# JeffreyXiang/ivid

Measured on NVIDIA H100. Metric: 128x128 RGBD multiview samples/sec, higher is better.
Workload: dtype fp16 tensor-core operands, fp32 accumulate / residual stream / GroupNorm / softmax / sampler

## Files before the change

ivid_b200/csrc/common.cuh:

```cuda
#pragma once
#include <cuda.h>
#include <cuda_fp16.h>
#include <cuda_fp8.h>
#include <cuda_runtime.h>
#include <stdint.h>

namespace ivid {

__device__ __forceinline__ uint32_t smem_u32(const void* p) {
  return static_cast<uint32_t>(__cvta_generic_to_shared(p));
}

__device__ __forceinline__ float silu_f(float x) {
  float e, r;
  asm("ex2.approx.ftz.f32 %0, %1;" : "=f"(e) : "f"(x * -1.4426950408889634f));
  asm("rcp.approx.ftz.f32 %0, %1;" : "=f"(r) : "f"(1.0f + e));
  return x * r;
}

__device__ __forceinline__ __half split_term(float v, int seg) {
  const __half hi = __float2half_rn(v);
  return seg == 1 ? __float2half_rn(v - __half2float(hi)) : hi;
}

// ... 34 lines not shown
    if (++spins > IVID_MBAR_SPIN_LIMIT) { __trap(); }
  }
}

__device__ __forceinline__ void bulk_load_1d(void* dst, const void* src, uint32_t bytes, uint64_t* bar) {
  asm volatile("cp.async.bulk.shared::cluster.global.mbarrier::complete_tx::bytes [%0], [%1], %2, [%3];\n" ::"r"(smem_u32(dst)),
               "l"(src), "r"(bytes), "r"(smem_u32(bar))
               : "memory");
}

__device__ __forceinline__ void tma_prefetch_desc(const CUtensorMap* m) {
  asm volatile("prefetch.tensormap [%0];\n" ::"l"(reinterpret_cast<uint64_t>(m)) : "memory");
}
__device__ __forceinline__ void tma_load_2d(const CUtensorMap* m, uint64_t* bar, void* dst, int c0, int c1) {
  asm volatile(
      "cp.async.bulk.tensor.2d.shared::cluster.global.mbarrier::complete_tx::bytes [%0], [%1, {%3, %4}], [%2];\n"
      ::"r"(smem_u32(dst)), "l"(reinterpret_cast<uint64_t>(m)), "r"(smem_u32(bar)), "r"(c0), "r"(c1)
      : "memory");
}
__device__ __forceinline__ void tma_load_3d(const CUtensorMap* m, uint64_t* bar, void* dst, int c0, int c1, int c2) {
  asm volatile(
      "cp.async.bulk.tensor.3d.shared::cluster.global.mbarrier::complete_tx::bytes [%0], [%1, {%3, %4, %5}], [%2];\n"
      ::"r"(smem_u32(dst)), "l"(reinterpret_cast<uint64_t>(m)), "r"(smem_u32(bar)), "r"(c0), "r"(c1), "r"(c2)
      : "memory");
}
__device__ __forceinline__ void tma_load_4d(const CUtensorMap* m, uint64_t* bar, void* dst, int c0, int c1, int c2,
                                            int c3) {
  asm volatile(
      "cp.async.bulk.tensor.4d.shared::cluster.global.mbarrier::complete_tx::bytes [%0], [%1, {%3, %4, %5, %6}], "
      "[%2];\n" ::"r"(smem_u32(dst)),
      "l"(reinterpret_cast<uint64_t>(m)), "r"(smem_u32(bar)), "r"(c0), "r"(c1), "r"(c2), "r"(c3)
      : "memory");
}

__device__ __forceinline__ void wgmma_fence() { asm volatile("wgmma.fence.sync.aligned;\n" ::: "memory"); }
__device__ __forceinline__ void wgmma_commit() { asm volatile("wgmma.commit_group.sync.aligned;\n" ::: "memory"); }
template <int kPending>
__device__ __forceinline__ void wgmma_wait() { asm volatile("wgmma.wait_group.sync.aligned %0;\n" ::"n"(kPending) : "memory"); }
template <int R>
__device__ __forceinline__ void reg_fence(float (&d)[R]) {
#pragma unroll
  for (int i = 0; i < R; ++i) asm volatile("" : "+f"(d[i])::"memory");
}

__device__ __forceinline__ uint64_t make_smem_desc_sw128(uint32_t smem_addr, uint32_t sbo_bytes, uint32_t lbo_bytes) {
  uint64_t d = 0;
  d |= static_cast<uint64_t>((smem_addr & 0x3FFFF) >> 4);
  d |= static_cast<uint64_t>((lbo_bytes >> 4) & 0x3FFF) << 16;
  d |= static_cast<uint64_t>((sbo_bytes >> 4) & 0x3FFF) << 32;
  d |= static_cast<uint64_t>(1) << 62;
  return d;
}

template <int N>
__device__ void wgmma_ss(float (&d)[N / 2], uint64_t desc_a, uint64_t desc_b, uint32_t scale_d);
template <int N>
__device__ void wgmma_rs_tb(float (&d)[N / 2], const uint32_t (&a)[4], uint64_t desc_b, uint32_t scale_d);
template <>
__device__ __forceinline__ void wgmma_ss<16>(float (&d)[8], uint64_t desc_a, uint64_t desc_b, uint32_t scale_d) {
  asm volatile(
      "{\n\t.reg .pred p;\n\tsetp.ne.b32 p, %10, 0;\n\t"
      "wgmma.mma_async.sync.aligned.m64n16k16.f32.f16.f16 {%0, %1, %2, %3, %4, %5, %6, %7}, %8, %9, p, 1, 1, 0, 0;\n\t}\n"
      : "+f"(d[0]), "+f"(d[1]), "+f"(d[2]), "+f"(d[3]), "+f"(d[4]), "+f"(d[5]), "+f"(d[6]), "+f"(d[7])
      : "l"(desc_a), "l"(desc_b), "r"(scale_d));
}
template <>
// ... 64 lines not shown
```

ivid_b200/csrc/conv_gemm.cuh:

```cuda
#pragma once
#include <type_traits>

#include "common.cuh"

namespace ivid {

struct ConvGemmParams {
  int N, H, W;
  int TW, TH, TN;
  int tiles_w, tiles_h, tiles_n;
  int n_blocks;
  int seg_chunks[3];
  int seg_taps[3];
  int Cout;
  int ldc;
  int ldr;
  int out_mode;
  const float* bias;
  const float* residual;
  int res_up;
  void* out;
  __half* out16;
  double* stats;
  float acc_scale;
};

struct ConvMaps {
  CUtensorMap a[3];
  CUtensorMap b;
};
struct ConvMaps8 : ConvMaps {
  CUtensorMap b8;
};

template <int BN, bool SLAB = false>
struct ConvGemmCfg {
  static constexpr int BM = 128;
  static constexpr int BK = 64;
  static constexpr int A_BYTES = BM * BK * 2;
  static constexpr int B_BYTES = ((BN * BK * 2 + 1023) / 1024) * 1024;
  static constexpr int STAGE_BYTES = A_BYTES + B_BYTES;
  static constexpr int STAGES = BN == 128 && !SLAB ? 3 : 4;
  static constexpr int SLAB_BYTES = 16 * 10 * 128;
  static constexpr int SLAB_STAGES = 2;
  static constexpr int RING_BYTES = SLAB ? SLAB_STAGES * SLAB_BYTES + STAGES * B_BYTES : STAGES * STAGE_BYTES;
  static constexpr int BAR_BYTES = 128;
  static constexpr int STAT_BYTES = 8 * 2 * BN * 4;
  static constexpr bool STATS_ON_RING = SLAB;
  static constexpr int SMEM_BYTES = RING_BYTES + BAR_BYTES + (STATS_ON_RING ? 0 : STAT_BYTES) + 1024;
  static constexpr int CONSUMER_THREADS = 256;
  static constexpr int THREADS = CONSUMER_THREADS + 32;
};

struct ConvKCursor {
  int seg = 0, t = 0, ch = 0, base = 0;
};

template <int BN, bool A8 = false, bool SLAB = false>
__global__ void __launch_bounds__(ConvGemmCfg<BN>::THREADS, 2)
conv_gemm_kernel(const __grid_constant__ std::conditional_t<A8, ConvMaps8, ConvMaps> maps, const __grid_constant__ ConvGemmParams p) {
  using Cfg = ConvGemmCfg<BN, SLAB>;
  constexpr int STAGES = Cfg::STAGES;
  constexpr int SLAB_STAGES = Cfg::SLAB_STAGES;
  extern __shared__ uint8_t smem_raw[];
  uint8_t* smem = smem_raw + ((1024u - (smem_u32(smem_raw) & 1023u)) & 1023u);
  uint64_t* full_bar = reinterpret_cast<uint64_t*>(smem + Cfg::RING_BYTES);
  uint64_t* empty_bar = full_bar + STAGES;
  uint64_t* slab_full = empty_bar + STAGES;
  uint64_t* slab_empty = slab_full + SLAB_STAGES;
  float* stat_smem = reinterpret_cast<float*>(Cfg::STATS_ON_RING ? smem : smem + Cfg::RING_BYTES + Cfg::BAR_BYTES);
  uint8_t* const slab_ring = smem;
  uint8_t* const w_ring = smem + SLAB_STAGES * Cfg::SLAB_BYTES;

  const int tid = threadIdx.x;
  const int warp = tid >> 5, lane = tid & 31;
  const int wg = warp >> 2;

  if (tid == 0) {
    for (int s = 0; s < STAGES; ++s) {
      mbar_init(&full_bar[s], 1);
      mbar_init(&empty_bar[s], 8u);
    }
    if constexpr (SLAB) {
      for (int s = 0; s < SLAB_STAGES; ++s) {
        mbar_init(&slab_full[s], 1);
        mbar_init(&slab_empty[s], 8u);
      }
    }
    fence_barrier_init();
  }
  __syncthreads();

  int nunits = 0;
  for (int sg = 0; sg < 3; ++sg) nunits += p.seg_chunks[sg] * p.seg_taps[sg];
  const int nunits8 = A8 ? p.seg_chunks[0] * p.seg_taps[0] : 0;

  const int mt = static_cast<int>(blockIdx.x) / p.n_blocks, nb = static_cast<int>(blockIdx.x) % p.n_blocks;
  const int colbase = nb * BN;
  const int tiles_per_img = p.tiles_w * p.tiles_h;
  const int tn = mt / tiles_per_img;
  const int rem = mt - tn * tiles_per_img;
  const int th = rem / p.tiles_w;
  const int tw = rem - th * p.tiles_w;
  const int n0 = tn * p.TN, h0 = th * p.TH, w0 = tw * p.TW;

  if (warp == Cfg::CONSUMER_THREADS / 32) {
    if (lane == 0) {
      tma_prefetch_desc(&maps.a[0]);
      tma_prefetch_desc(&maps.b);
      if constexpr (A8) tma_prefetch_desc(&maps.b8);
      if constexpr (SLAB) {
        const uint32_t slab_bytes = static_cast<uint32_t>(p.TW * (p.TH + 2)) * 128u;
        uint32_t u = 0, a = 0;
        int base = 0;
#pragma unroll 1
        for (int sg = 0; sg < 3; ++sg) {
          const int chunks = p.seg_chunks[sg];
          const int nx = p.seg_taps[sg] == 9 ? 3 : 1;
          const bool e4m3 = A8 && sg == 0;
#pragma unroll 1
          for (int ch = 0; ch < chunks; ++ch) {
#pragma unroll 1
            for (int xi = 0; xi < nx; ++xi, ++a) {
              const int sl = static_cast<int>(a % SLAB_STAGES);
              if (a >= SLAB_STAGES) mbar_wait(&slab_empty[sl], ((a / SLAB_STAGES) - 1) & 1);
              mbar_arrive_expect_tx(&slab_full[sl], nx == 3 ? slab_bytes : static_cast<uint32_t>(Cfg::A_BYTES));
              tma_load_4d(&maps.a[sg], &slab_full[sl], slab_ring + sl * Cfg::SLAB_BYTES, ch * (e4m3 ? 128 : 64),
                          w0 + (nx == 3 ? xi - 1 : 0), h0 - (nx == 3 ? 1 : 0), n0);
#pragma unroll 1
              for (int yi = 0; yi < nx; ++yi, ++u) {
                const int s = static_cast<int>(u % STAGES);
                if (u >= STAGES) mbar_wait(&empty_bar[s], ((u / STAGES) - 1) & 1);
                mbar_arrive_expect_tx(&full_bar[s], BN * Cfg::BK * 2);
                const int t = nx == 3 ? 3 * yi + xi : 0;
                uint8_t* sb = w_ring + s * Cfg::B_BYTES;
                if constexpr (A8) {
                  if (e4m3) { tma_load_2d(&maps.b8, &full_bar[s], sb, (t * chunks + ch) * 128, colbase); continue; }
                }
                tma_load_2d(&maps.b, &full_bar[s], sb, base + (t * chunks + ch) * 64, colbase);
              }
            }
          }
          if (!e4m3) base += p.seg_taps[sg] * chunks * 64;
// ... 2 lines not shown
        ConvKCursor c;
        while (p.seg_chunks[c.seg] == 0) ++c.seg;
#pragma unroll 1
        for (int u = 0; u < nunits; ++u) {
          const uint32_t g = static_cast<uint32_t>(u);
          const int s = static_cast<int>(g % STAGES);
          if (g >= STAGES) mbar_wait(&empty_bar[s], ((g / STAGES) - 1) & 1);
          const int taps = p.seg_taps[c.seg], chunks = p.seg_chunks[c.seg];
          uint8_t* sa = smem + s * Cfg::STAGE_BYTES;
          uint8_t* sb = sa + Cfg::A_BYTES;
          const int dy = (taps == 9) ? (c.t / 3 - 1) : 0;
          const int dx = (taps == 9) ? (c.t % 3 - 1) : 0;
          mbar_arrive_expect_tx(&full_bar[s], Cfg::A_BYTES + BN * Cfg::BK * 2);
          bool e4m3 = false;
          if constexpr (A8) {
            if (c.seg == 0) {
              tma_load_4d(&maps.a[0], &full_bar[s], sa, c.ch * 128, w0 + dx, h0 + dy, n0);
              tma_load_2d(&maps.b8, &full_bar[s], sb, (c.t * chunks + c.ch) * 128, colbase);
              e4m3 = true;
            }
          }
          if (!e4m3) {
            const int kcol = c.base + (c.t * chunks + c.ch) * 64;
            tma_load_4d(&maps.a[c.seg], &full_bar[s], sa, c.ch * 64, w0 + dx, h0 + dy, n0);
            tma_load_2d(&maps.b, &full_bar[s], sb, kcol, colbase);
          }
          if (++c.ch == chunks) {
            c.ch = 0;
            if (++c.t == taps) { c.t = 0; if (!A8 || c.seg != 0) c.base += taps * chunks * 64; ++c.seg; }
          }
          while (c.seg < 3 && p.seg_chunks[c.seg] == 0) ++c.seg;
        }
      }
    }
    return;
  }

  float acc[BN / 2];
#pragma unroll
  for (int i = 0; i < BN / 2; ++i) acc[i] = 0.f;

  if constexpr (SLAB) {
    const uint32_t row_bytes = static_cast<uint32_t>(p.TW) * 128u;
    uint32_t u = 0, a = 0;
#pragma unroll 1
    for (int sg = 0; sg < 3; ++sg) {
      const int nx = p.seg_taps[sg] == 9 ? 3 : 1;
      const int loads = p.seg_chunks[sg] * nx;
#pragma unroll 1
      for (int l = 0; l < loads; ++l, ++a) {
        const uint32_t sl = a % SLAB_STAGES;
        mbar_wait(&slab_full[sl], (a / SLAB_STAGES) & 1);
        const uint32_t sa = smem_u32(slab_ring + sl * Cfg::SLAB_BYTES) + wg * 64 * 128;
#pragma unroll 1
        for (int yi = 0; yi < nx; ++yi, ++u) {
          const uint32_t s = u % STAGES;
          mbar_wait(&full_bar[s], (u / STAGES) & 1);
          wgmma_fence();
          const uint64_t da = make_smem_desc_sw128(sa + yi * row_bytes, 1024, 16);
          const uint64_t db = make_smem_desc_sw128(smem_u32(w_ring + s * Cfg::B_BYTES), 1024, 16);
          if (A8 && sg == 0) {
#pragma unroll
            for (int k = 0; k < 4; ++k) wgmma_ss_e4m3<BN>(acc, da + 2 * k, db + 2 * k, (u | k) != 0 ? 1u : 0u);
          } else {
#pragma unroll
            for (int k = 0; k < 4; ++k) wgmma_ss<BN>(acc, da + 2 * k, db + 2 * k, (u | k) != 0 ? 1u : 0u);
// ... 12 lines not shown
    if (lane == 0) {
      mbar_arrive(&empty_bar[(u - 1) % STAGES]);
      mbar_arrive(&slab_empty[(a - 1) % SLAB_STAGES]);
    }
  } else {
#pragma unroll 1
    for (int u = 0; u < nunits; ++u) {
      const uint32_t g = static_cast<uint32_t>(u);
      const int s = static_cast<int>(g % STAGES);
      mbar_wait(&full_bar[s], (g / STAGES) & 1);
      const uint32_t sa = smem_u32(smem + s * Cfg::STAGE_BYTES);
      const uint32_t sb = sa + Cfg::A_BYTES;
      wgmma_fence();
      const uint64_t da = make_smem_desc_sw128(sa + wg * 64 * 128, 1024, 16);
      const uint64_t db = make_smem_desc_sw128(sb, 1024, 16);
      if (A8 && u < nunits8) {
#pragma unroll
        for (int k = 0; k < 4; ++k) wgmma_ss_e4m3<BN>(acc, da + 2 * k, db + 2 * k, (u | k) != 0 ? 1u : 0u);
      } else {
#pragma unroll
        for (int k = 0; k < 4; ++k) wgmma_ss<BN>(acc, da + 2 * k, db + 2 * k, (u | k) != 0 ? 1u : 0u);
      }
      wgmma_commit();
      wgmma_wait<1>();
      if (u > 0 && lane == 0) mbar_arrive(&empty_bar[(g - 1) % STAGES]);
    }
    wgmma_wait<0>();
    reg_fence(acc);
    if (lane == 0) mbar_arrive(&empty_bar[static_cast<uint32_t>(nunits - 1) % STAGES]);
  }

  const int wr = warp & 3;
  const int quad = lane & 3;
  uint32_t pix[2], rpix[2];
  bool ok[2];
#pragma unroll
  for (int i = 0; i < 2; ++i) {
    const int row = wg * 64 + wr * 16 + (lane >> 2) + 8 * i;
    const int n = n0 + row / (p.TW * p.TH), h = h0 + (row / p.TW) % p.TH, x = w0 + row % p.TW;
    ok[i] = n < p.N;
    pix[i] = (static_cast<uint32_t>(n) * p.H + h) * p.W + x;
    rpix[i] = p.res_up ? (static_cast<uint32_t>(n) * (p.H >> 1) + (h >> 1)) * (p.W >> 1) + (x >> 1) : pix[i];
  }
  const bool do_stats = p.stats != nullptr;
  if constexpr (Cfg::STATS_ON_RING) {
    if (do_stats) asm volatile("bar.sync 1, %0;\n" ::"n"(Cfg::CONSUMER_THREADS) : "memory");
  }
#pragma unroll
  for (int j = 0; j < BN / 8; ++j) {
    const int c = colbase + 8 * j + 2 * quad;
    float s0 = 0.f, s1 = 0.f, q0 = 0.f, q1 = 0.f;
    if (c < p.Cout) {
      const float2 b = make_float2(__ldg(p.bias + c), __ldg(p.bias + c + 1));
#pragma unroll
      for (int i = 0; i < 2; ++i) {
        if (!ok[i]) continue;
        float v0, v1;
        if (A8) {
          v0 = fmaf(acc[4 * j + 2 * i], p.acc_scale, b.x); v1 = fmaf(acc[4 * j + 2 * i + 1], p.acc_scale, b.y);
        } else {
          v0 = acc[4 * j + 2 * i] + b.x; v1 = acc[4 * j + 2 * i + 1] + b.y;
        }
        if (p.out_mode == 2) {
          const uint32_t hw = static_cast<uint32_t>(p.H) * p.W, n = pix[i] / hw;
          float* o = reinterpret_cast<float*>(p.out) + (static_cast<size_t>(n) * p.Cout + c) * hw + (pix[i] - n * hw);
          o[0] = v0;
          if (c + 1 < p.Cout) o[hw] = v1;
          continue;
        }
        if (p.residual != nullptr) {
          const float2 r = __ldg(reinterpret_cast<const float2*>(p.residual + static_cast<size_t>(rpix[i]) * p.ldr + c));
          v0 += r.x; v1 += r.y;
        }
        if (p.out_mode == 0) {
          *reinterpret_cast<float2*>(reinterpret_cast<float*>(p.out) + static_cast<size_t>(pix[i]) * p.ldc + c) = make_float2(v0, v1);
          if (p.out16 != nullptr) *reinterpret_cast<uint32_t*>(p.out16 + static_cast<size_t>(pix[i]) * p.ldc + c) = pack_h2(v0, v1);
        } else {
          const __half2 hv = __floats2half2_rn(v0, v1);
          *reinterpret_cast<__half2*>(reinterpret_cast<__half*>(p.out) + static_cast<size_t>(pix[i]) * p.ldc + c) = hv;
          const float2 r = __half22float2(hv);
          v0 = r.x; v1 = r.y;
        }
        s0 += v0; s1 += v1;
        q0 = fmaf(v0, v0, q0); q1 = fmaf(v1, v1, q1);
      }
    }
    if (do_stats) {
#pragma unroll
      for (int off = 4; off < 32; off <<= 1) {
        s0 += __shfl_xor_sync(0xffffffffu, s0, off);
        s1 += __shfl_xor_sync(0xffffffffu, s1, off);
        q0 += __shfl_xor_sync(0xffffffffu, q0, off);
        q1 += __shfl_xor_sync(0xffffffffu, q1, off);
      }
      if (lane < 4) {
        float* st = stat_smem + warp * 2 * BN + 8 * j + 2 * quad;
        st[0] = s0; st[1] = s1; st[BN] = q0; st[BN + 1] = q1;
      }
    }
  }
  if (do_stats) {
    asm volatile("bar.sync 1, %0;\n" ::"n"(Cfg::CONSUMER_THREADS) : "memory");
    const int rows_per_n = p.TW * p.TH;
    const int n_tile = (128 + rows_per_n - 1) / rows_per_n;
    for (int e = tid; e < n_tile * BN; e += Cfg::CONSUMER_THREADS) {
      const int sn = e / BN, c = e - sn * BN;
      const int n = n0 + sn, col = colbase + c;
      if (n >= p.N || col >= p.Cout) continue;
      float ssum = 0.f, qsum = 0.f;
      for (int w8 = 0; w8 < 8; ++w8) {
        if ((w8 * 16) / rows_per_n != sn) continue;
        ssum += stat_smem[w8 * 2 * BN + c];
        qsum += stat_smem[w8 * 2 * BN + BN + c];
      }
      double* st = p.stats + (static_cast<size_t>(n) * p.Cout + col) * 2;
      atomicAdd(st, static_cast<double>(ssum));
      atomicAdd(st + 1, static_cast<double>(qsum));
    }
  }
}

}
```

ivid_b200/csrc/host_util.cu:

```cuda
#include "host_util.h"

#include <cmath>
#include <cstring>
#include <mutex>

namespace ivid {

typedef CUresult (*PFN_encodeTiled)(CUtensorMap*, CUtensorMapDataType, cuuint32_t, void*, const cuuint64_t*,
                                    const cuuint64_t*, const cuuint32_t*, const cuuint32_t*, CUtensorMapInterleave,
                                    CUtensorMapSwizzle, CUtensorMapL2promotion, CUtensorMapFloatOOBfill);

static PFN_encodeTiled get_encode_fn() {
  static PFN_encodeTiled fn = nullptr;
  static std::once_flag once;
  std::call_once(once, [] {
    void* p = nullptr;
    cudaDriverEntryPointQueryResult qres;
    cudaError_t e = cudaGetDriverEntryPoint("cuTensorMapEncodeTiled", &p, cudaEnableDefault, &qres);
    if (e == cudaSuccess && qres == cudaDriverEntryPointSuccess) fn = reinterpret_cast<PFN_encodeTiled>(p);
  });
  if (!fn) throw Error(kErrCuda, "cuTensorMapEncodeTiled is not available from the CUDA driver");
  return fn;
}

CUtensorMap make_tensor_map(CUtensorMapDataType dtype, int rank, void* base, const uint64_t* dims,
                            const uint64_t* strides_bytes, const uint32_t* box, CUtensorMapSwizzle swizzle) {
  CUtensorMap m;
  std::memset(&m, 0, sizeof(m));
  cuuint64_t gdims[5];
  cuuint64_t gstr[4];
  cuuint32_t bx[5];
  cuuint32_t es[5];
  for (int i = 0; i < rank; ++i) {
    gdims[i] = dims[i];
    bx[i] = box[i];
    es[i] = 1;
  }
  for (int i = 0; i + 1 < rank; ++i) gstr[i] = strides_bytes[i];
  CUresult r = get_encode_fn()(&m, dtype, static_cast<cuuint32_t>(rank), base, gdims, gstr, bx, es,
                               CU_TENSOR_MAP_INTERLEAVE_NONE, swizzle, CU_TENSOR_MAP_L2_PROMOTION_L2_256B,
                               CU_TENSOR_MAP_FLOAT_OOB_FILL_NONE);
  if (r != CUDA_SUCCESS) {
    throw Error(kErrCuda, "cuTensorMapEncodeTiled failed with CUresult " + std::to_string(static_cast<int>(r)));
  }
  return m;
}

static uint64_t elem_bytes(CUtensorMapDataType dtype) { return dtype == CU_TENSOR_MAP_DATA_TYPE_UINT8 ? 1 : 2; }

CUtensorMap make_act_map(const void* base, int N, int H, int W, int C, int TW, int TH, int TN, CUtensorMapDataType dtype) {
  const uint64_t es = elem_bytes(dtype);
  const uint64_t dims[4] = {static_cast<uint64_t>(C), static_cast<uint64_t>(W), static_cast<uint64_t>(H),
                            static_cast<uint64_t>(N)};
  const uint64_t str[3] = {static_cast<uint64_t>(C) * es, static_cast<uint64_t>(W) * C * es,
                           static_cast<uint64_t>(H) * W * C * es};
  const uint32_t box[4] = {static_cast<uint32_t>(128 / es), static_cast<uint32_t>(TW), static_cast<uint32_t>(TH),
                           static_cast<uint32_t>(TN)};
  return make_tensor_map(dtype, 4, const_cast<void*>(base), dims, str, box, CU_TENSOR_MAP_SWIZZLE_128B);
}

CUtensorMap make_weight_map(const void* base, int rows, int K, int box_rows, CUtensorMapDataType dtype) {
  const uint64_t es = elem_bytes(dtype);
  const uint64_t dims[2] = {static_cast<uint64_t>(K), static_cast<uint64_t>(rows)};
  const uint64_t str[1] = {static_cast<uint64_t>(K) * es};
  const uint32_t box[2] = {static_cast<uint32_t>(128 / es), static_cast<uint32_t>(box_rows)};
  return make_tensor_map(dtype, 2, const_cast<void*>(base), dims, str, box, CU_TENSOR_MAP_SWIZZLE_128B);
}

int sm_count() {
  static int n = 0;
  if (n == 0) {
    int dev = 0;
    if (cudaGetDevice(&dev) != cudaSuccess) return 132;
    cudaDeviceProp prop;
    if (cudaGetDeviceProperties(&prop, dev) != cudaSuccess) return 132;
    n = prop.multiProcessorCount;
  }
  return n;
}

uint8_t fp8_e4m3_from_float(float v) {
  uint32_t bits;
  std::memcpy(&bits, &v, 4);
  const uint8_t sign = static_cast<uint8_t>((bits >> 24) & 0x80u);
  if ((bits & 0x7FFFFFFFu) > 0x7F800000u) return sign | 0x7F;
  const double a = std::fabs(static_cast<double>(v));
  if (a >= 448.0) return sign | 0x7E;
  if (a < 0.015625) {
    return sign | static_cast<uint8_t>(std::nearbyint(a * 512.0));
  }
  int k;
// ... 24 lines not shown
```

ivid_b200/csrc/host_util.h:

```cpp
#pragma once
#include <cuda.h>
#include <cuda_runtime.h>
#include <stdint.h>

#include <stdexcept>
#include <string>

namespace ivid {

struct Error : std::runtime_error {
  int code;
  Error(int c, const std::string& m) : std::runtime_error(m), code(c) {}
};

enum : int {
  kOk = 0,
  kErrInvalidArgument = 1,
  kErrNotImplemented = 2,
  kErrCuda = 3,
  kErrState = 4,
};

#define IVID_CHECK_CUDA(expr)                                                                              \
  do {                                                                                                     \
    cudaError_t _e = (expr);                                                                               \
    if (_e != cudaSuccess)                                                                                 \
      throw ::ivid::Error(::ivid::kErrCuda, std::string(#expr) + " failed: " + cudaGetErrorString(_e) +   \
                                                " (" __FILE__ ":" + std::to_string(__LINE__) + ")");       \
  } while (0)

#define IVID_REQUIRE(cond, msg)                                                      \
  do {                                                                               \
    if (!(cond)) throw ::ivid::Error(::ivid::kErrInvalidArgument, std::string(msg)); \
  } while (0)

CUtensorMap make_tensor_map(CUtensorMapDataType dtype, int rank, void* base, const uint64_t* dims,
                            const uint64_t* strides_bytes , const uint32_t* box,
                            CUtensorMapSwizzle swizzle);

CUtensorMap make_act_map(const void* base, int N, int H, int W, int C, int TW, int TH, int TN,
                         CUtensorMapDataType dtype = CU_TENSOR_MAP_DATA_TYPE_FLOAT16);
CUtensorMap make_weight_map(const void* base, int rows, int K, int box_rows,
                            CUtensorMapDataType dtype = CU_TENSOR_MAP_DATA_TYPE_FLOAT16);

int sm_count();

uint8_t fp8_e4m3_from_float(float v);
float fp8_e4m3_to_float(uint8_t q);
int fp8_weight_exponent(float max_abs);

}
```

ivid_b200/csrc/ops.cu:

```cuda
#include "ops.h"

#include <algorithm>
#include <cmath>
#include <mutex>

#include "attention.cuh"
#include "attention_hd.cuh"
#include "conv_gemm.cuh"
#include "elementwise.cuh"
#include "embed.cuh"

namespace ivid {

struct ConvLaunch {
  ConvMaps8 maps;
  ConvGemmParams p;
  int BN;
  bool a8;
  bool slab;
  int grid;
};

int conv_pad_cout(int cout) {
  if (cout >= 64) return ((cout + 63) / 64) * 64;
  return ((cout + 15) / 16) * 16;
}
static int pow2_divisor(int v, int cap) {
  int t = 1;
  while (t * 2 <= cap && v % (t * 2) == 0) t *= 2;
  return t;
}
void conv_tile(int H, int W, int* TW, int* TH, int* TN) {
  IVID_REQUIRE(H > 0 && W > 0, "conv: spatial size must be positive");
  *TW = pow2_divisor(W, 16);
  *TH = pow2_divisor(H, 128 / *TW);
  *TN = 128 / (*TW * *TH);
}
bool conv_can_fuse_stats(int H, int W) {
  int TW, TH, TN;
  conv_tile(H, W, &TW, &TH, &TN);
  return TW * TH >= 32;
}
int conv_pick_bn(int cout_pad) {
  if (cout_pad % 128 == 0) return 128;
  if (cout_pad % 64 == 0) return 64;
  if (cout_pad % 16 == 0 && cout_pad <= 48) return 16;
  throw Error(kErrInvalidArgument, "conv: unsupported padded Cout " + std::to_string(cout_pad));
}

bool conv_can_res_up(int W, int cout) { return W >= 16 && cout % 8 == 0; }
bool conv_can_out16(int cout) { return cout % 8 == 0; }
int conv_pad_k(int c) { return ((c + 63) / 64) * 64; }
int conv_pad_k8(int c) { return ((c + 127) / 128) * 128; }
int conv_seg_cols(int taps, int c) { return taps * conv_pad_k(c); }

ConvPack conv_pack(const float* w, const float* b, int cout, int cin, int ksz, int pitch, const float* w2, const float* b2,
                   int cin2, int cin2a, bool e4m3) {
  ConvPack pk;
  const int taps = ksz * ksz;
  pk.cout_pad = conv_pad_cout(cout);
  float scale = 1.f;
  if (e4m3) {
    IVID_REQUIRE(pitch == conv_pad_k(cin), "internal: an e4m3 segment 0 is an ordinary 3x3 or 1x1 conv");
    float mx = 0.f;
    for (size_t i = 0; i < static_cast<size_t>(cout) * cin * taps; ++i) mx = std::max(mx, std::fabs(w[i]));
    const int e = fp8_weight_exponent(mx);
    const float kMinNormal16 = std::ldexp(1.0f, -14);
    if (cin % 16 != 0) pk.refused = "its input channels are not a multiple of 16";
    else if (e < -100 || e > 100) pk.refused = "its weight exponent is outside [-100, 100]";
    for (size_t i = 0; pk.refused == nullptr && i < static_cast<size_t>(cout) * cin2; ++i) {
      const float v = std::fabs(w2[i]), sv = v * std::ldexp(1.0f, e);
      if (sv > 65504.f) pk.refused = "its skip weights times 2^e overflow fp16";
      else if (v >= kMinNormal16 && sv < kMinNormal16) pk.refused = "its skip weights times 2^e become fp16 subnormals";
    }
    pk.e4m3 = pk.refused == nullptr;
    if (pk.e4m3) { pk.e = e; scale = std::ldexp(1.0f, e); }
  }
  const int s0 = cin2a > 0 ? cin2a : cin2, s1 = cin2 - s0;
  const int k0 = pk.e4m3 ? 0 : conv_seg_cols(1, taps * pitch);
  pk.K = k0 + conv_seg_cols(1, s0) + conv_seg_cols(1, s1);
  pk.w16.assign(static_cast<size_t>(pk.cout_pad) * pk.K, __float2half_rn(0.f));
  const int cp8 = conv_pad_k8(cin), K8 = pk.e4m3 ? taps * cp8 : 0;
  pk.w8.assign(static_cast<size_t>(pk.cout_pad) * K8, 0);
  for (int co = 0; co < cout; ++co) {
    __half* row = pk.w16.data() + static_cast<size_t>(co) * pk.K;
    for (int tap = 0; tap < taps; ++tap)
      for (int ci = 0; ci < cin; ++ci) {
        const float v = w[(static_cast<size_t>(co) * cin + ci) * taps + tap];
        if (pk.e4m3) pk.w8[static_cast<size_t>(co) * K8 + tap * cp8 + ci] = fp8_e4m3_from_float(v * scale);
        else row[tap * pitch + ci] = __float2half_rn(v);
      }
    for (int ci = 0; ci < cin2; ++ci)
      row[k0 + (ci < s0 ? ci : conv_pad_k(s0) + ci - s0)] = __float2half_rn(w2[static_cast<size_t>(co) * cin2 + ci] * scale);
  }
  pk.bias.assign(pk.cout_pad, 0.f);
  for (int i = 0; i < cout; ++i) {
    if (b != nullptr) pk.bias[i] = b[i];
    if (b2 != nullptr) pk.bias[i] += b2[i];
  }
  return pk;
}

ConvLaunch* conv_launch_create(const ConvDesc& d) {
  IVID_REQUIRE(d.C0 > 0 && d.C0 % 8 == 0, "conv: segment-0 channels must be a positive multiple of 8");
  IVID_REQUIRE(d.C1 % 8 == 0, "conv: segment-1 channels must be a multiple of 8");
  IVID_REQUIRE(d.taps0 == 9 || d.taps0 == 1, "conv: only 3x3 (pad 1) and 1x1 kernels are on this path");
  IVID_REQUIRE(d.taps1 == 9 || d.taps1 == 1, "conv: only 3x3 (pad 1) and 1x1 kernels are on this path");
  IVID_REQUIRE(d.C2 % 8 == 0 && (d.taps2 == 9 || d.taps2 == 1), "conv: segment 2 must be a multiple of 8 channels, 3x3 or 1x1");
  IVID_REQUIRE(d.N > 0 && static_cast<int64_t>(d.N) * d.H * d.W < (int64_t{1} << 31),
               "conv: N*H*W must be below 2^31 (32-bit pixel indices in the epilogue)");
  const bool a8 = d.weight8 != nullptr;
  IVID_REQUIRE(!a8 || d.C0 % 16 == 0, "conv: an e4m3 segment 0 needs a multiple of 16 channels (16-byte TMA rows)");
  auto* l = new ConvLaunch();
  l->a8 = a8;
  ConvGemmParams& p = l->p;
  p.N = d.N; p.H = d.H; p.W = d.W;
  conv_tile(d.H, d.W, &p.TW, &p.TH, &p.TN);
  p.tiles_w = d.W / p.TW;
  p.tiles_h = d.H / p.TH;
  p.tiles_n = (d.N + p.TN - 1) / p.TN;
  const bool any3x3 = d.taps0 == 9 || (d.C1 > 0 && d.taps1 == 9) || (d.C2 > 0 && d.taps2 == 9);
  l->slab = any3x3 && p.TN == 1 && p.TW >= 8;
  IVID_REQUIRE(!l->slab || p.TW * (p.TH + 2) * 128 <= (ConvGemmCfg<128, true>::SLAB_BYTES), "internal: conv slab larger than its slot");
  l->BN = conv_pick_bn(d.cout_pad);
  p.n_blocks = d.cout_pad / l->BN;
  p.seg_chunks[0] = a8 ? conv_pad_k8(d.C0) / 128 : conv_pad_k(d.C0) / 64; p.seg_taps[0] = d.taps0;
  p.acc_scale = d.acc_scale;
  p.seg_chunks[1] = conv_pad_k(d.C1) / 64; p.seg_taps[1] = d.C1 > 0 ? d.taps1 : 0;
  p.seg_chunks[2] = conv_pad_k(d.C2) / 64; p.seg_taps[2] = d.C2 > 0 ? d.taps2 : 0;
  p.Cout = d.cout; p.ldc = d.ldc; p.ldr = d.ldr; p.out_mode = d.out_mode;
  p.bias = d.bias; p.residual = d.residual; p.out = d.out;
  p.stats = (d.stats != nullptr && conv_can_fuse_stats(d.H, d.W) && d.out_mode != 2) ? d.stats : nullptr;
  IVID_REQUIRE(d.stats == nullptr || p.stats != nullptr, "conv: fused statistics need >= 32 pixels per sample per warp");
  IVID_REQUIRE(d.out_mode == 2 || (d.cout % 8 == 0 && d.ldc % 8 == 0), "conv: NHWC output needs Cout % 8 == 0");
  IVID_REQUIRE(d.residual == nullptr || (d.out_mode != 2 && d.ldr % 2 == 0), "conv: residual needs an NHWC output and an even row pitch");
  p.res_up = 0;
  if (d.residual != nullptr && d.residual_up) {
    IVID_REQUIRE(conv_can_res_up(d.W, d.cout) && d.H % 2 == 0, "conv: upsampled residual needs W >= 16 and Cout % 8 == 0");
    p.res_up = 1;
  }
  p.out16 = nullptr;
  if (d.out16 != nullptr) {
    IVID_REQUIRE(d.out_mode == 0 && conv_can_out16(d.cout), "conv: fp16 output copy needs an fp32 NHWC output and Cout % 8 == 0");
    p.out16 = static_cast<__half*>(d.out16);
  }
  const int Ktot = (a8 ? 0 : conv_seg_cols(d.taps0, d.C0)) + conv_seg_cols(d.taps1, d.C1) + conv_seg_cols(d.taps2, d.C2);
  ConvMaps8& M = l->maps;
  auto rows = [&](int taps) { return l->slab && taps == 9 ? p.TH + 2 : p.TH; };
  M.a[0] = a8 ? make_act_map(d.act0, d.N, d.H, d.W, d.C0, p.TW, rows(d.taps0), p.TN, CU_TENSOR_MAP_DATA_TYPE_UINT8)
              : make_act_map(d.act0, d.N, d.H, d.W, d.C0, p.TW, rows(d.taps0), p.TN);
  M.a[1] = d.C1 > 0 ? make_act_map(d.act1, d.N, d.H, d.W, d.C1, p.TW, rows(d.taps1), p.TN) : M.a[0];
  M.a[2] = d.C2 > 0 ? make_act_map(d.act2, d.N, d.H, d.W, d.C2, p.TW, rows(d.taps2), p.TN) : M.a[0];
  if (a8) {
    M.b8 = make_weight_map(d.weight8, d.cout_pad, d.taps0 * conv_pad_k8(d.C0), l->BN, CU_TENSOR_MAP_DATA_TYPE_UINT8);
    M.b = Ktot > 0 ? make_weight_map(d.weight, d.cout_pad, Ktot, l->BN) : M.b8;
  } else {
    M.b = make_weight_map(d.weight, d.cout_pad, Ktot, l->BN);
  }
  l->grid = p.tiles_w * p.tiles_h * p.tiles_n * p.n_blocks;
  return l;
}
void conv_launch_destroy(ConvLaunch* l) { delete l; }
int conv_launch_bn(const ConvLaunch* l) { return l->BN; }
bool conv_launch_a8(const ConvLaunch* l) { return l->a8; }

template <int BN, bool A8, bool SLAB>
static void run_conv(const ConvLaunch* l, cudaStream_t s) {
  using Cfg = ConvGemmCfg<BN, SLAB>;
  static std::once_flag once;
  std::call_once(once, [] {
    IVID_CHECK_CUDA(cudaFuncSetAttribute(conv_gemm_kernel<BN, A8, SLAB>, cudaFuncAttributeMaxDynamicSharedMemorySize, Cfg::SMEM_BYTES));
  });
  if constexpr (A8) conv_gemm_kernel<BN, true, SLAB><<<l->grid, Cfg::THREADS, Cfg::SMEM_BYTES, s>>>(l->maps, l->p);
  else conv_gemm_kernel<BN, false, SLAB><<<l->grid, Cfg::THREADS, Cfg::SMEM_BYTES, s>>>(static_cast<const ConvMaps&>(l->maps), l->p);
  IVID_CHECK_CUDA(cudaGetLastError());
}
template <bool A8, bool SLAB>
static void run_conv_bn(const ConvLaunch* l, cudaStream_t s) {
  switch (l->BN) {
    case 128: run_conv<128, A8, SLAB>(l, s); break;
    case 64: run_conv<64, A8, SLAB>(l, s); break;
    default: run_conv<16, A8, SLAB>(l, s); break;
  }
}
void conv_launch_run_out(const ConvLaunch* l, void* out, cudaStream_t s) {
  ConvLaunch tmp = *l;
  tmp.p.out = out;
  conv_launch_run(&tmp, s);
}
void conv_launch_run(const ConvLaunch* l, cudaStream_t s) {
  if (l->a8) {
    if (l->slab) run_conv_bn<true, true>(l, s);
    else run_conv_bn<true, false>(l, s);
  } else {
    if (l->slab) run_conv_bn<false, true>(l, s);
    else run_conv_bn<false, false>(l, s);
  }
}

struct AttnLaunch {
  CUtensorMap mapQ, mapKV;
  AttnParams p;
  AttnHdParams hp;
  int head_ch = 64;
  int nv = 0;
  bool qres = false;
  int smem = 0;
  int grid;
};

AttnLaunch* attn_launch_create(const void* qkv, int N, int T, int C, int head_ch, void* out) {
  if (head_ch <= 0 || head_ch % 64 != 0)
    throw Error(kErrNotImplemented, "attention: head width " + std::to_string(head_ch) + " is not a multiple of 64");
  IVID_REQUIRE(C % head_ch == 0, "attention: channels must be a multiple of the head width " + std::to_string(head_ch));
  IVID_REQUIRE(T >= 1, "attention: sequence length must be positive");
  auto* l = new AttnLaunch();
  l->head_ch = head_ch;
  l->p.N = N; l->p.T = T; l->p.C = C; l->p.heads = C / 64;
// ... 214 lines not shown
```

Before: 0.3250.

## Stage conv epilogue through shared memory with TMA residual loads and output stores

Reworks the conv GEMM epilogue so the producer warp TMA-loads the fp32 residual tile into freed ring slots (with an L2 prefetch at kernel start). Consumers add bias and residual from shared memory, write the fp32 and fp16 outputs into swizzled shared-memory tiles, and one thread issues bulk TMA tensor stores. This replaces scattered per-thread float2 global loads and stores with coalesced bulk transfers. The cost is extra barriers, ring-slot reuse constraints, new 16-byte alignment requirements, and run-time output patching restricted to NCHW.

```diff
diff --git a/ivid_b200/csrc/common.cuh b/ivid_b200/csrc/common.cuh
--- a/ivid_b200/csrc/common.cuh
+++ b/ivid_b200/csrc/common.cuh
@@ -90,6 +90,19 @@
       "l"(reinterpret_cast<uint64_t>(m)), "r"(smem_u32(bar)), "r"(c0), "r"(c1), "r"(c2), "r"(c3)
       : "memory");
 }
+__device__ __forceinline__ void tma_prefetch_l2_4d(const CUtensorMap* m, int c0, int c1, int c2, int c3) {
+  asm volatile("cp.async.bulk.prefetch.tensor.4d.L2.global.tile [%0, {%1, %2, %3, %4}];\n" ::"l"(reinterpret_cast<uint64_t>(m)),
+               "r"(c0), "r"(c1), "r"(c2), "r"(c3)
+               : "memory");
+}
+__device__ __forceinline__ void tma_store_4d(const CUtensorMap* m, const void* src, int c0, int c1, int c2, int c3) {
+  asm volatile("cp.async.bulk.tensor.4d.global.shared::cta.bulk_group [%0, {%2, %3, %4, %5}], [%1];\n" ::"l"(
+                   reinterpret_cast<uint64_t>(m)),
+               "r"(smem_u32(src)), "r"(c0), "r"(c1), "r"(c2), "r"(c3)
+               : "memory");
+}
+__device__ __forceinline__ void tma_store_commit() { asm volatile("cp.async.bulk.commit_group;\n" ::: "memory"); }
+__device__ __forceinline__ void tma_store_wait_read() { asm volatile("cp.async.bulk.wait_group.read 0;\n" ::: "memory"); }
 
 __device__ __forceinline__ void wgmma_fence() { asm volatile("wgmma.fence.sync.aligned;\n" ::: "memory"); }
 __device__ __forceinline__ void wgmma_commit() { asm volatile("wgmma.commit_group.sync.aligned;\n" ::: "memory"); }
diff --git a/ivid_b200/csrc/conv_gemm.cuh b/ivid_b200/csrc/conv_gemm.cuh
--- a/ivid_b200/csrc/conv_gemm.cuh
+++ b/ivid_b200/csrc/conv_gemm.cuh
@@ -28,6 +28,9 @@
 struct ConvMaps {
   CUtensorMap a[3];
   CUtensorMap b;
+  CUtensorMap r;
+  CUtensorMap o;
+  CUtensorMap o16;
 };
 struct ConvMaps8 : ConvMaps {
   CUtensorMap b8;
@@ -50,6 +53,19 @@
   static constexpr int SMEM_BYTES = RING_BYTES + BAR_BYTES + (STATS_ON_RING ? 0 : STAT_BYTES) + 1024;
   static constexpr int CONSUMER_THREADS = 256;
   static constexpr int THREADS = CONSUMER_THREADS + 32;
+
+  static constexpr int F32_CH = SLAB ? BN / 4 : (BN < 32 ? BN : 32);
+  static constexpr int F32_BOX = BM * F32_CH * 4;
+  static constexpr int UNIT_BOXES = !SLAB && BN == 128 ? 2 : 1;
+  static constexpr int UNIT_CH = F32_CH * UNIT_BOXES;
+  static constexpr int UNITS = BN / UNIT_CH;
+  static constexpr int UNIT_STRIDE = SLAB ? B_BYTES : STAGE_BYTES;
+  static constexpr int F16_CH = BN < 64 ? BN : 64;
+  static constexpr int F16_BOX = BM * F16_CH * 2;
+  static constexpr int F16_TILE = BM * BN * 2;
+  static_assert(UNIT_BOXES * F32_BOX <= UNIT_STRIDE, "an fp32 unit must fit its ring slot");
+  static_assert(SLAB ? UNITS == STAGES : UNITS < STAGES && F16_TILE <= STAGE_BYTES, "fp32 units and the fp16 tile must fit the ring");
+  static_assert(!SLAB || F16_TILE + STAT_BYTES <= SLAB_STAGES * SLAB_BYTES, "the fp16 tile and statistics must fit the slab slots");
 };
 
 struct ConvKCursor {
@@ -68,7 +84,7 @@
   uint64_t* empty_bar = full_bar + STAGES;
   uint64_t* slab_full = empty_bar + STAGES;
   uint64_t* slab_empty = slab_full + SLAB_STAGES;
-  float* stat_smem = reinterpret_cast<float*>(Cfg::STATS_ON_RING ? smem : smem + Cfg::RING_BYTES + Cfg::BAR_BYTES);
+  float* stat_smem = reinterpret_cast<float*>(Cfg::STATS_ON_RING ? smem + Cfg::F16_TILE : smem + Cfg::RING_BYTES + Cfg::BAR_BYTES);
   uint8_t* const slab_ring = smem;
   uint8_t* const w_ring = smem + SLAB_STAGES * Cfg::SLAB_BYTES;
 
@@ -103,12 +119,18 @@
   const int th = rem / p.tiles_w;
   const int tw = rem - th * p.tiles_w;
   const int n0 = tn * p.TN, h0 = th * p.TH, w0 = tw * p.TW;
+  uint8_t* const unit_ring = SLAB ? w_ring : smem;
 
   if (warp == Cfg::CONSUMER_THREADS / 32) {
     if (lane == 0) {
+      const int rw0 = p.res_up ? w0 >> 1 : w0, rh0 = p.res_up ? h0 >> 1 : h0;
       tma_prefetch_desc(&maps.a[0]);
       tma_prefetch_desc(&maps.b);
       if constexpr (A8) tma_prefetch_desc(&maps.b8);
+      if (p.residual != nullptr) {
+#pragma unroll
+        for (int q = 0; q < Cfg::UNITS * Cfg::UNIT_BOXES; ++q) tma_prefetch_l2_4d(&maps.r, colbase + q * Cfg::F32_CH, rw0, rh0, n0);
+      }
       if constexpr (SLAB) {
         const uint32_t slab_bytes = static_cast<uint32_t>(p.TW * (p.TH + 2)) * 128u;
         uint32_t u = 0, a = 0;
@@ -177,6 +199,21 @@
           while (c.seg < 3 && p.seg_chunks[c.seg] == 0) ++c.seg;
         }
       }
+      if (p.residual != nullptr) {
+        const uint32_t bytes = static_cast<uint32_t>(Cfg::UNIT_BOXES * Cfg::F32_BOX) >> (p.res_up ? 2 : 0);
+#pragma unroll 1
+        for (int i = 0; i < Cfg::UNITS; ++i) {
+          const uint32_t g = static_cast<uint32_t>(nunits + i);
+          const int s = static_cast<int>(g % STAGES);
+          const int q = SLAB ? s : i;
+          if (g >= STAGES) mbar_wait(&empty_bar[s], ((g / STAGES) - 1) & 1);
+          mbar_arrive_expect_tx(&full_bar[s], bytes);
+#pragma unroll
+          for (int k = 0; k < Cfg::UNIT_BOXES; ++k)
+            tma_load_4d(&maps.r, &full_bar[s], unit_ring + s * Cfg::UNIT_STRIDE + k * Cfg::F32_BOX,
+                        colbase + q * Cfg::UNIT_CH + k * Cfg::F32_CH, rw0, rh0, n0);
+        }
+      }
     }
     return;
   }
@@ -255,55 +292,114 @@
 
   const int wr = warp & 3;
   const int quad = lane & 3;
-  uint32_t pix[2], rpix[2];
+  constexpr int RB32 = Cfg::F32_CH * 4, RB16 = Cfg::F16_CH * 2;
+  const uint32_t s_res = static_cast<uint32_t>(nunits) % STAGES;
+  auto row_base = [](uint32_t r, int rb) {
+    const uint32_t m = rb >= 128 ? 7u : rb == 64 ? 3u : rb == 32 ? 1u : 0u;
+    return r * rb ^ ((((r * rb) >> 7) & m) << 4);
+  };
+  const uint32_t units_u32 = smem_u32(unit_ring);
+  auto unit_at = [&](int u) { return units_u32 + (SLAB ? u : (s_res + u) % STAGES) * Cfg::UNIT_STRIDE; };
+  auto f32_at = [&](int j, uint32_t t) {
+    if constexpr (Cfg::F32_CH >= 8) {
+      const int cl = 8 * j;
+      return unit_at(cl / Cfg::UNIT_CH) + (cl % Cfg::UNIT_CH) / Cfg::F32_CH * Cfg::F32_BOX + (t ^ (cl % Cfg::F32_CH) * 4);
+    } else {
+      return unit_at(2 * j + (quad >> 1)) + t;
+    }
+  };
+  const int rows_per_n = p.TW * p.TH;
   bool ok[2];
 #pragma unroll
-  for (int i = 0; i < 2; ++i) {
-    const int row = wg * 64 + wr * 16 + (lane >> 2) + 8 * i;
-    const int n = n0 + row / (p.TW * p.TH), h = h0 + (row / p.TW) % p.TH, x = w0 + row % p.TW;
-    ok[i] = n < p.N;
-    pix[i] = (static_cast<uint32_t>(n) * p.H + h) * p.W + x;
-    rpix[i] = p.res_up ? (static_cast<uint32_t>(n) * (p.H >> 1) + (h >> 1)) * (p.W >> 1) + (x >> 1) : pix[i];
-  }
-  const bool do_stats = p.stats != nullptr;
-  if constexpr (Cfg::STATS_ON_RING) {
-    if (do_stats) asm volatile("bar.sync 1, %0;\n" ::"n"(Cfg::CONSUMER_THREADS) : "memory");
-  }
-#pragma unroll
-  for (int j = 0; j < BN / 8; ++j) {
-    const int c = colbase + 8 * j + 2 * quad;
-    float s0 = 0.f, s1 = 0.f, q0 = 0.f, q1 = 0.f;
-    if (c < p.Cout) {
-      const float2 b = make_float2(__ldg(p.bias + c), __ldg(p.bias + c + 1));
+  for (int i = 0; i < 2; ++i) ok[i] = n0 + (wg * 64 + wr * 16 + (lane >> 2) + 8 * i) / rows_per_n < p.N;
+
+  if (p.residual != nullptr) {
+#pragma unroll 1
+    for (int q = 0; q < Cfg::UNITS; ++q) {
+      const uint32_t g = static_cast<uint32_t>(nunits + q);
+      mbar_wait(&full_bar[g % STAGES], (g / STAGES) & 1);
+    }
+  }
+  {
+    uint32_t tr[2];
+#pragma unroll
+    for (int i = 0; i < 2; ++i) {
+      const int row = wg * 64 + wr * 16 + (lane >> 2) + 8 * i;
+      const int nl = row / rows_per_n, hl = (row / p.TW) % p.TH, xl = row % p.TW;
+      const uint32_t rr = p.res_up ? (nl * (p.TH >> 1) + (hl >> 1)) * (p.TW >> 1) + (xl >> 1) : row;
+      tr[i] = row_base(rr, RB32) ^ ((8 * quad) % RB32);
+    }
+    const float* bias = p.bias + colbase + 2 * quad;
+#pragma unroll
+    for (int j = 0; j < BN / 8; ++j) {
+      const float2 b = make_float2(__ldg(bias + 8 * j), __ldg(bias + 8 * j + 1));
 #pragma unroll
       for (int i = 0; i < 2; ++i) {
-        if (!ok[i]) continue;
         float v0, v1;
         if (A8) {
           v0 = fmaf(acc[4 * j + 2 * i], p.acc_scale, b.x); v1 = fmaf(acc[4 * j + 2 * i + 1], p.acc_scale, b.y);
         } else {
           v0 = acc[4 * j + 2 * i] + b.x; v1 = acc[4 * j + 2 * i + 1] + b.y;
         }
-        if (p.out_mode == 2) {
-          const uint32_t hw = static_cast<uint32_t>(p.H) * p.W, n = pix[i] / hw;
-          float* o = reinterpret_cast<float*>(p.out) + (static_cast<size_t>(n) * p.Cout + c) * hw + (pix[i] - n * hw);
-          o[0] = v0;
-          if (c + 1 < p.Cout) o[hw] = v1;
-          continue;
-        }
         if (p.residual != nullptr) {
-          const float2 r = __ldg(reinterpret_cast<const float2*>(p.residual + static_cast<size_t>(rpix[i]) * p.ldr + c));
-          v0 += r.x; v1 += r.y;
-        }
-        if (p.out_mode == 0) {
-          *reinterpret_cast<float2*>(reinterpret_cast<float*>(p.out) + static_cast<size_t>(pix[i]) * p.ldc + c) = make_float2(v0, v1);
-          if (p.out16 != nullptr) *reinterpret_cast<uint32_t*>(p.out16 + static_cast<size_t>(pix[i]) * p.ldc + c) = pack_h2(v0, v1);
-        } else {
-          const __half2 hv = __floats2half2_rn(v0, v1);
-          *reinterpret_cast<__half2*>(reinterpret_cast<__half*>(p.out) + static_cast<size_t>(pix[i]) * p.ldc + c) = hv;
-          const float2 r = __half22float2(hv);
-          v0 = r.x; v1 = r.y;
-        }
+          float r0, r1;
+          asm volatile("ld.shared.v2.f32 {%0, %1}, [%2];\n" : "=f"(r0), "=f"(r1) : "r"(f32_at(j, tr[i])) : "memory");
+          v0 += r0; v1 += r1;
+        }
+        acc[4 * j + 2 * i] = v0; acc[4 * j + 2 * i + 1] = v1;
+      }
+    }
+  }
+
+  if (p.out_mode == 2) {
+    const uint32_t hw = static_cast<uint32_t>(p.H) * p.W;
+#pragma unroll
+    for (int i = 0; i < 2; ++i) {
+      if (!ok[i]) continue;
+      const int row = wg * 64 + wr * 16 + (lane >> 2) + 8 * i;
+      const int nl = row / rows_per_n, hl = (row / p.TW) % p.TH, xl = row % p.TW;
+      float* o = reinterpret_cast<float*>(p.out) + (static_cast<size_t>(n0 + nl) * p.Cout + colbase + 2 * quad) * hw +
+                 static_cast<uint32_t>(h0 + hl) * p.W + (w0 + xl);
+#pragma unroll
+      for (int j = 0; j < BN / 8; ++j, o += 8 * static_cast<size_t>(hw)) {
+        const int c = colbase + 8 * j + 2 * quad;
+        if (c >= p.Cout) continue;
+        o[0] = acc[4 * j + 2 * i];
+        if (c + 1 < p.Cout) o[hw] = acc[4 * j + 2 * i + 1];
+      }
+    }
+    return;
+  }
+  asm volatile("bar.sync 1, %0;\n" ::"n"(Cfg::CONSUMER_THREADS) : "memory");
+
+  const uint32_t f16_u32 = SLAB ? smem_u32(slab_ring) : smem_u32(smem) + ((s_res + Cfg::UNITS) % STAGES) * Cfg::STAGE_BYTES;
+  uint32_t t32[2], t16[2];
+#pragma unroll
+  for (int i = 0; i < 2; ++i) {
+    const uint32_t row = wg * 64 + wr * 16 + (lane >> 2) + 8 * i;
+    t32[i] = row_base(row, RB32) ^ ((8 * quad) % RB32);
+    t16[i] = row_base(row, RB16) ^ (4 * quad);
+  }
+  const bool do_stats = p.stats != nullptr;
+  const int c_left = p.Cout - (colbase + 2 * quad);
+  const uint32_t st_u32 = smem_u32(stat_smem) + (warp * 2 * BN + 2 * quad) * 4;
+#pragma unroll
+  for (int j = 0; j < BN / 8; ++j) {
+    float s0 = 0.f, s1 = 0.f, q0 = 0.f, q1 = 0.f;
+#pragma unroll
+    for (int i = 0; i < 2; ++i) {
+      float v0 = acc[4 * j + 2 * i], v1 = acc[4 * j + 2 * i + 1];
+      const uint32_t a16 = f16_u32 + (8 * j) / Cfg::F16_CH * Cfg::F16_BOX + (t16[i] ^ ((8 * j) % Cfg::F16_CH) * 2);
+      if (p.out_mode == 0) {
+        asm volatile("st.shared.v2.f32 [%0], {%1, %2};\n" ::"r"(f32_at(j, t32[i])), "f"(v0), "f"(v1) : "memory");
+        if (p.out16 != nullptr) asm volatile("st.shared.b32 [%0], %1;\n" ::"r"(a16), "r"(pack_h2(v0, v1)) : "memory");
+      } else {
+        const __half2 hv = __floats2half2_rn(v0, v1);
+        asm volatile("st.shared.b32 [%0], %1;\n" ::"r"(a16), "r"(*reinterpret_cast<const uint32_t*>(&hv)) : "memory");
+        const float2 r = __half22float2(hv);
+        v0 = r.x; v1 = r.y;
+      }
+      if (ok[i] && 8 * j < c_left) {
         s0 += v0; s1 += v1;
         q0 = fmaf(v0, v0, q0); q1 = fmaf(v1, v1, q1);
       }
@@ -317,14 +413,34 @@
         q1 += __shfl_xor_sync(0xffffffffu, q1, off);
       }
       if (lane < 4) {
-        float* st = stat_smem + warp * 2 * BN + 8 * j + 2 * quad;
-        st[0] = s0; st[1] = s1; st[BN] = q0; st[BN + 1] = q1;
-      }
-    }
+        const uint32_t st = st_u32 + 32 * j;
+        asm volatile("st.shared.v2.f32 [%0], {%1, %2};\n" ::"r"(st), "f"(s0), "f"(s1) : "memory");
+        asm volatile("st.shared.v2.f32 [%0], {%1, %2};\n" ::"r"(st + 4 * BN), "f"(q0), "f"(q1) : "memory");
+      }
+    }
+  }
+  fence_proxy_async_smem();
+  asm volatile("bar.sync 1, %0;\n" ::"n"(Cfg::CONSUMER_THREADS) : "memory");
+  if (tid == 0) {
+    if (p.out_mode == 0) {
+#pragma unroll
+      for (int q = 0; q < Cfg::UNITS * Cfg::UNIT_BOXES; ++q) {
+        const int u = q / Cfg::UNIT_BOXES, k = q % Cfg::UNIT_BOXES;
+        const int col = colbase + q * Cfg::F32_CH;
+        if (col < p.Cout)
+          tma_store_4d(&maps.o, unit_ring + (SLAB ? u : (s_res + u) % STAGES) * Cfg::UNIT_STRIDE + k * Cfg::F32_BOX, col, w0, h0, n0);
+      }
+    }
+    if (p.out_mode == 1 || p.out16 != nullptr) {
+#pragma unroll
+      for (int q = 0; q < BN / Cfg::F16_CH; ++q) {
+        const int col = colbase + q * Cfg::F16_CH;
+        if (col < p.Cout) tma_store_4d(&maps.o16, (SLAB ? slab_ring : smem + ((s_res + Cfg::UNITS) % STAGES) * Cfg::STAGE_BYTES) + q * Cfg::F16_BOX, col, w0, h0, n0);
+      }
+    }
+    tma_store_commit();
   }
   if (do_stats) {
-    asm volatile("bar.sync 1, %0;\n" ::"n"(Cfg::CONSUMER_THREADS) : "memory");
-    const int rows_per_n = p.TW * p.TH;
     const int n_tile = (128 + rows_per_n - 1) / rows_per_n;
     for (int e = tid; e < n_tile * BN; e += Cfg::CONSUMER_THREADS) {
       const int sn = e / BN, c = e - sn * BN;
@@ -341,6 +457,7 @@
       atomicAdd(st + 1, static_cast<double>(qsum));
     }
   }
+  if (tid == 0) tma_store_wait_read();
 }
 
 }
diff --git a/ivid_b200/csrc/host_util.cu b/ivid_b200/csrc/host_util.cu
--- a/ivid_b200/csrc/host_util.cu
+++ b/ivid_b200/csrc/host_util.cu
@@ -46,17 +46,26 @@
   return m;
 }
 
-static uint64_t elem_bytes(CUtensorMapDataType dtype) { return dtype == CU_TENSOR_MAP_DATA_TYPE_UINT8 ? 1 : 2; }
+static uint64_t elem_bytes(CUtensorMapDataType dtype) {
+  return dtype == CU_TENSOR_MAP_DATA_TYPE_UINT8 ? 1 : dtype == CU_TENSOR_MAP_DATA_TYPE_FLOAT32 ? 4 : 2;
+}
 
-CUtensorMap make_act_map(const void* base, int N, int H, int W, int C, int TW, int TH, int TN, CUtensorMapDataType dtype) {
+CUtensorMap make_act_map(const void* base, int N, int H, int W, int C, int TW, int TH, int TN, CUtensorMapDataType dtype,
+                         int pitch, int box_c) {
   const uint64_t es = elem_bytes(dtype);
+  const uint64_t ld = static_cast<uint64_t>(pitch > 0 ? pitch : C);
+  if (box_c <= 0) box_c = static_cast<int>(128 / es);
   const uint64_t dims[4] = {static_cast<uint64_t>(C), static_cast<uint64_t>(W), static_cast<uint64_t>(H),
                             static_cast<uint64_t>(N)};
-  const uint64_t str[3] = {static_cast<uint64_t>(C) * es, static_cast<uint64_t>(W) * C * es,
-                           static_cast<uint64_t>(H) * W * C * es};
-  const uint32_t box[4] = {static_cast<uint32_t>(128 / es), static_cast<uint32_t>(TW), static_cast<uint32_t>(TH),
+  const uint64_t str[3] = {ld * es, static_cast<uint64_t>(W) * ld * es, static_cast<uint64_t>(H) * W * ld * es};
+  const uint32_t box[4] = {static_cast<uint32_t>(box_c), static_cast<uint32_t>(TW), static_cast<uint32_t>(TH),
                            static_cast<uint32_t>(TN)};
-  return make_tensor_map(dtype, 4, const_cast<void*>(base), dims, str, box, CU_TENSOR_MAP_SWIZZLE_128B);
+  const uint64_t row = static_cast<uint64_t>(box_c) * es;
+  const CUtensorMapSwizzle sw = row == 128 ? CU_TENSOR_MAP_SWIZZLE_128B
+                                : row == 64 ? CU_TENSOR_MAP_SWIZZLE_64B
+                                : row == 32 ? CU_TENSOR_MAP_SWIZZLE_32B
+                                            : CU_TENSOR_MAP_SWIZZLE_NONE;
+  return make_tensor_map(dtype, 4, const_cast<void*>(base), dims, str, box, sw);
 }
 
 CUtensorMap make_weight_map(const void* base, int rows, int K, int box_rows, CUtensorMapDataType dtype) {
diff --git a/ivid_b200/csrc/host_util.h b/ivid_b200/csrc/host_util.h
--- a/ivid_b200/csrc/host_util.h
+++ b/ivid_b200/csrc/host_util.h
@@ -39,7 +39,7 @@
                             CUtensorMapSwizzle swizzle);
 
 CUtensorMap make_act_map(const void* base, int N, int H, int W, int C, int TW, int TH, int TN,
-                         CUtensorMapDataType dtype = CU_TENSOR_MAP_DATA_TYPE_FLOAT16);
+                         CUtensorMapDataType dtype = CU_TENSOR_MAP_DATA_TYPE_FLOAT16, int pitch = 0, int box_c = 0);
 CUtensorMap make_weight_map(const void* base, int rows, int K, int box_rows,
                             CUtensorMapDataType dtype = CU_TENSOR_MAP_DATA_TYPE_FLOAT16);
 
diff --git a/ivid_b200/csrc/ops.cu b/ivid_b200/csrc/ops.cu
--- a/ivid_b200/csrc/ops.cu
+++ b/ivid_b200/csrc/ops.cu
@@ -48,7 +48,7 @@
   throw Error(kErrInvalidArgument, "conv: unsupported padded Cout " + std::to_string(cout_pad));
 }
 
-bool conv_can_res_up(int W, int cout) { return W >= 16 && cout % 8 == 0; }
+bool conv_can_res_up(int W, int cout) { return W >= 16 && W % 2 == 0 && cout % 8 == 0; }
 bool conv_can_out16(int cout) { return cout % 8 == 0; }
 int conv_pad_k(int c) { return ((c + 63) / 64) * 64; }
 int conv_pad_k8(int c) { return ((c + 127) / 128) * 128; }
@@ -99,6 +99,19 @@
     if (b2 != nullptr) pk.bias[i] += b2[i];
   }
   return pk;
+}
+
+template <int BN, bool SLAB>
+static void epilogue_box_channels(int* f32_ch, int* f16_ch) {
+  *f32_ch = ConvGemmCfg<BN, SLAB>::F32_CH;
+  *f16_ch = ConvGemmCfg<BN, SLAB>::F16_CH;
+}
+static void epilogue_box_channels(int BN, bool slab, int* f32_ch, int* f16_ch) {
+  switch (BN) {
+    case 128: slab ? epilogue_box_channels<128, true>(f32_ch, f16_ch) : epilogue_box_channels<128, false>(f32_ch, f16_ch); break;
+    case 64: slab ? epilogue_box_channels<64, true>(f32_ch, f16_ch) : epilogue_box_channels<64, false>(f32_ch, f16_ch); break;
+    default: slab ? epilogue_box_channels<16, true>(f32_ch, f16_ch) : epilogue_box_channels<16, false>(f32_ch, f16_ch); break;
+  }
 }
 
 ConvLaunch* conv_launch_create(const ConvDesc& d) {
@@ -133,12 +146,16 @@
   p.stats = (d.stats != nullptr && conv_can_fuse_stats(d.H, d.W) && d.out_mode != 2) ? d.stats : nullptr;
   IVID_REQUIRE(d.stats == nullptr || p.stats != nullptr, "conv: fused statistics need >= 32 pixels per sample per warp");
   IVID_REQUIRE(d.out_mode == 2 || (d.cout % 8 == 0 && d.ldc % 8 == 0), "conv: NHWC output needs Cout % 8 == 0");
-  IVID_REQUIRE(d.residual == nullptr || (d.out_mode != 2 && d.ldr % 2 == 0), "conv: residual needs an NHWC output and an even row pitch");
+  IVID_REQUIRE(d.residual == nullptr || (d.out_mode != 2 && d.ldr % 4 == 0 && d.ldr >= d.cout),
+               "conv: residual needs an NHWC output and a row pitch of >= Cout, a multiple of 4 elements");
   p.res_up = 0;
   if (d.residual != nullptr && d.residual_up) {
-    IVID_REQUIRE(conv_can_res_up(d.W, d.cout) && d.H % 2 == 0, "conv: upsampled residual needs W >= 16 and Cout % 8 == 0");
+    IVID_REQUIRE(conv_can_res_up(d.W, d.cout) && d.H % 2 == 0, "conv: upsampled residual needs an even W >= 16 and Cout % 8 == 0");
     p.res_up = 1;
   }
+  auto aligned = [](const void* q) { return (reinterpret_cast<uintptr_t>(q) & 15u) == 0; };
+  IVID_REQUIRE(d.out_mode == 2 || (aligned(d.out) && aligned(d.out16) && aligned(d.residual)),
+               "conv: NHWC output, fp16 copy and residual must be 16-byte aligned");
   p.out16 = nullptr;
   if (d.out16 != nullptr) {
     IVID_REQUIRE(d.out_mode == 0 && conv_can_out16(d.cout), "conv: fp16 output copy needs an fp32 NHWC output and Cout % 8 == 0");
@@ -157,6 +174,17 @@
   } else {
     M.b = make_weight_map(d.weight, d.cout_pad, Ktot, l->BN);
   }
+  int f32_ch = 0, f16_ch = 0;
+  epilogue_box_channels(l->BN, l->slab, &f32_ch, &f16_ch);
+  const auto f32 = CU_TENSOR_MAP_DATA_TYPE_FLOAT32;
+  M.r = M.o = M.o16 = M.a[0];
+  if (d.residual != nullptr) {
+    const int up = p.res_up ? 1 : 0;
+    M.r = make_act_map(d.residual, d.N, d.H >> up, d.W >> up, d.cout, p.TW >> up, p.TH >> up, p.TN, f32, d.ldr, f32_ch);
+  }
+  if (d.out_mode == 0) M.o = make_act_map(d.out, d.N, d.H, d.W, d.cout, p.TW, p.TH, p.TN, f32, d.ldc, f32_ch);
+  const void* o16 = d.out_mode == 1 ? d.out : d.out_mode == 0 ? d.out16 : nullptr;
+  if (o16 != nullptr) M.o16 = make_act_map(o16, d.N, d.H, d.W, d.cout, p.TW, p.TH, p.TN, CU_TENSOR_MAP_DATA_TYPE_FLOAT16, d.ldc, f16_ch);
   l->grid = p.tiles_w * p.tiles_h * p.tiles_n * p.n_blocks;
   return l;
 }
@@ -184,6 +212,7 @@
   }
 }
 void conv_launch_run_out(const ConvLaunch* l, void* out, cudaStream_t s) {
+  IVID_REQUIRE(l->p.out_mode == 2, "internal: only an NCHW conv output is patched at run time (NHWC outputs are in tensor maps)");
   ConvLaunch tmp = *l;
   tmp.p.out = out;
   conv_launch_run(&tmp, s);
```

After: 0.3562, median of 6. 9.6% higher.
